# pqh22/ProxyTransformation

Measured on AMD Instinct MI355X. Metric: scenes/sec (100k pts, 256 clusters, 64 proxies), higher is better.
Workload: dtype f32; 1 GPU; cfg2: N=100000 pts, gs=8->M'=256 kept clusters, L=64 text + V=196 image proxies, d=256, eval forward; scenes_per_gpu=4, img_feat_dtype=bf16, input_sets_rotated=3, streams=1, lanes=1 (one forward at a time), setup_forwards=32

## Files before the change

### proxytransformation_amd/csrc/api.hip

```cpp
#include <atomic>
#include <chrono>
#include <cmath>
#include <cstdlib>
#include <cstring>
#include <mutex>
#include <utility>
#include <vector>

#include "common.h"

namespace ptx {

static thread_local char g_err[512] = "";

void set_error(const char *fmt, ...)
{
    va_list ap;
    va_start(ap, fmt);
    vsnprintf(g_err, sizeof(g_err), fmt, ap);
    va_end(ap);
}

static const char *const kKernelNames[] = {
    "k_minmax", "k_cluster", "k_select", "k_tags",
// ... 977 lines not shown
    PTX_REQUIRE(points && tag && kcenter && translate && transform && out && counts, "ptx_affine_compact: null argument");
    PTX_TRY(check_bufs(s, workspace, ws_bytes));
    hipStream_t st = static_cast<hipStream_t>(stream);
    int32_t *tc = at<int32_t>(workspace, ws_layout(*s).tile_counts);
    PTX_TRY(launch_tile_count(tag, s->B, s->N, tc, counts, nullptr, st));
    ScenePts sp;
    PTX_TRY(make_scene_pts(points, nullptr, s->B, s->N, &sp));
    return launch_affine(*s, sp, const_cast<uint32_t *>(tag), kcenter, translate, transform, out, counts, tc, true, false, st);
}

#define PTX_DBG(field, src, bytes)                                                                         do {                                                                                                       if (debug && debug->field)                                                                                 PTX_HIP(hipMemcpyAsync(debug->field, src, bytes, hipMemcpyDeviceToDevice, st));                } while (0)

int ptx_forward(PtxContext *ctx, const PtxShape *s, const PtxWeights *w, const void *prep, const float *lin,
                const float *points, const float *const *points_list, const float *text_feats,
                const uint8_t *text_mask, const void *img_feat, const int32_t *order_override,
                const float *centers_override,
                float *out, int32_t *counts, void *workspace, size_t ws_bytes, const PtxDebug *debug,
                void *stream)
{
    return ptx_forward_ex(ctx, s, w, prep, lin, points, points_list, text_feats, text_mask, img_feat, order_override,
                          centers_override, out, counts, workspace, ws_bytes, debug, nullptr, stream);
}

int ptx_forward_ex(PtxContext *ctx, const PtxShape *s, const PtxWeights *w, const void *prep, const float *lin,
                   const float *points, const float *const *points_list, const float *text_feats,
                   const uint8_t *text_mask, const void *img_feat, const int32_t *order_override,
                   const float *centers_override,
                   float *out, int32_t *counts, void *workspace, size_t ws_bytes, const PtxDebug *debug,
                   const PtxForwardOpts *opts, void *stream)
{
    PTX_REQUIRE(w && prep && lin && (points || points_list) && text_feats && img_feat && out && counts,
                "ptx_forward: null argument");
    const uint32_t *bbox_in = opts ? opts->bbox_enc : nullptr;
    const int compute_dtype = opts ? opts->compute_dtype : 0;
    PTX_REQUIRE(compute_dtype == 0 || compute_dtype == 1, "ptx_forward: compute_dtype=%d (0 fp32-equivalent, 1 bf16)", compute_dtype);
    PTX_TRY(check_bufs(s, workspace, ws_bytes));
    ScenePts sp;
    PTX_TRY(make_scene_pts(points, points_list, s->B, s->N, &sp));
    hipStream_t st = static_cast<hipStream_t>(stream);
    const PtxShape &S = *s;
    const PrepLayout P = prep_layout(S);
    const WsLayout L = ws_layout(S);
    const float *pf = static_cast<const float *>(prep);
    void *ws = workspace;
    const int M = S.grid_size * S.grid_size * S.grid_size, B = S.B, K = S.K, Kd = S.Mt - S.Mk;

    PtxContext *side = ctx;
    if (side == nullptr) PTX_TRY(default_context(&side));
    {
        int dev = 0;
        PTX_HIP(hipGetDevice(&dev));
        PTX_REQUIRE(dev == side->dev, "ptx_forward: context belongs to device %d, current device is %d", side->dev, dev);
    }
    std::lock_guard<std::mutex> enqueue_lock(side->mu);
    hipStreamCaptureStatus cap_status = hipStreamCaptureStatusNone;
    PTX_HIP(hipStreamIsCapturing(st, &cap_status));
    const bool capturing = cap_status != hipStreamCaptureStatusNone;
    if (!capturing) {
        PTX_TRY(gate_check(side));
        side->last_st = st; side->have_last = true;
        if (side->gates_on && (!side->probed || side->probed_st != st)) PTX_TRY(gate_probe(side, st));
    }
    const LayoutChoice lc = choose_layout(S);
    const double est_cluster = lc.est_cluster, est_image = lc.est_image;
    const LayoutForce &lf = lc.lf;
    const bool cluster_on_caller = lc.cluster_on_caller;
    hipStream_t cs = cluster_on_caller ? st : side->st, is = cluster_on_caller ? side->st : st;
    const bool gated = side->gates_on && !cluster_on_caller && !capturing;
    const bool img_late = lc.img_late;
    if (!gated && !img_late) {
        PTX_HIP(hipEventRecord(side->fork, st));
        PTX_HIP(hipStreamWaitEvent(side->st, side->fork, 0));
    }
    float *img_proxy = at<float>(ws, L.img_proxy);
#ifdef PTX_TEST_HOOKS
    static const char *const fault = getenv("PTX_GATE_FAULT");
#else
    constexpr const char *fault = nullptr;
#endif
    const bool fault_fork = gated && fault && fault[0] == 'f', fault_join = gated && fault && fault[0] == 'j';
    auto launch_gate = [&](int kid, hipStream_t s_, const GateRef &g) -> int {
        hipLaunchKernelGGL(k_gate, dim3(1), dim3(64), 0, s_, g);
        PTX_LAUNCHED("k_gate");
        (void)kid;
        return PTX_OK;
    };
    if (gated) {
        const uint32_t seq = ++side->gate_seq;
        PTX_TRY(run_img_proxy(S, *w, pf, img_feat, img_proxy, ws, is, 1, true, 0, -1, fault_fork ? nullptr : side->gate, seq));
        PTX_TIMED(KID_GATE_FORK, cs, launch_gate(KID_GATE_FORK, cs, gate_ref(side, 0, seq, 1)));
    } else
    if (!img_late) PTX_TRY(run_img_proxy(S, *w, pf, img_feat, img_proxy, ws, is, 1));

    uint32_t *mm_ws = at<uint32_t>(ws, L.mm_enc), *tag = at<uint32_t>(ws, L.tag);
    const uint32_t *mm_enc = bbox_in ? bbox_in : mm_ws;
    const bool dbg = debug != nullptr;
    float *centers0 = dbg && debug->centers0 ? at<float>(ws, L.centers0) : nullptr;
    float *cluster1 = dbg && debug->cluster1 ? at<float>(ws, L.cluster1) : nullptr;
    float *offsets = dbg && debug->offsets ? at<float>(ws, L.offsets) : nullptr;
    float *centers = at<float>(ws, L.centers), *cluster2 = at<float>(ws, L.cluster2);
    int32_t *idx2 = at<int32_t>(ws, L.idx2), *pad_count = at<int32_t>(ws, L.pad_count);
    if (!bbox_in) PTX_TIMED(KID_MINMAX, cs, launch_minmax(sp, B, S.N, mm_ws, cs));
    const bool early = lc.early;
    const bool fork_ext = !capturing && (img_late || early);
    const bool cgate = cluster_on_caller && side->gates_on && side->lo_ok && !capturing;
    if (cgate) ++side->gate_seq;
    const bool fault_cjoin = cgate && fault && fault[0] == 'j', fault_ctags = cgate && fault && fault[0] == 't';
    const bool cg_join_select = cgate && early;
    const bool cg_join_qkv = cgate && !early;
    GateRef cjoin = (cg_join_select || cg_join_qkv) ? gate_ref(side, 52, side->gate_seq, 2) : GateRef{};
    PTX_TIMED(KID_CLUSTER, cs, launch_cluster(S, mm_enc, lin, sp, pf + P.off_ab, w->offset, w->offset_map_w,
                                              centers_override, nullptr, centers0, cluster1, offsets, centers, idx2,
                                              cluster2, pad_count, cs, fork_ext ? side->early_a : nullptr));

    if (img_late) {
        if (!fork_ext) PTX_HIP(hipEventRecord(side->fork, st));
        PTX_HIP(hipStreamWaitEvent(side->st, fork_ext ? side->early_a : side->fork, 0));
        PTX_TRY(run_img_proxy(S, *w, pf, img_feat, img_proxy, ws, is, 1));
    }
    float *point_proxy = at<float>(ws, L.point_proxy);
    float *xin_t = at<float>(ws, L.x_in[0]), *xin_i = at<float>(ws, L.x_in[1]);
    float *translate = at<float>(ws, L.head[0]), *transform = at<float>(ws, L.head[1]);
    float *guide_t = (debug && debug->text_guide) ? at<float>(ws, L.guide[0]) : nullptr;
    float *guide_i = (debug && debug->img_guide) ? at<float>(ws, L.guide[1]) : nullptr;
    Branch br[2] = {make_branch(S, *w, pf, 0, xin_t, text_feats, S.L, text_mask, translate, guide_t),
                    make_branch(S, *w, pf, 1, xin_i, at<float>(ws, L.cbuf), S.V, nullptr, transform, guide_i)};
    br[1].proxy_lnp = at<float>(ws, L.lnp_img);
    if (early) {
        if (!fork_ext) PTX_HIP(hipEventRecord(side->early_a, cs));
        PTX_HIP(hipStreamWaitEvent(side->lo, side->early_a, 0));
        float *pp_all = at<float>(ws, L.pp_all), *xa_t = at<float>(ws, L.xln_all[0]), *xa_i = at<float>(ws, L.xln_all[1]);
        int32_t *order_e = at<int32_t>(ws, L.order_e);
        PTX_TRY(launch_order(S, pad_count, order_override, order_e, side->lo));
        PTX_TRY(launch_pointnet(pf + P.enc_ab, w->encoder, centers, cluster2, B * S.Mt, S.Mt, K, S.C, pp_all, &w->text, &w->img, nullptr,
                                nullptr, xa_t, xa_i, S.ln_eps, order_e, M, side->lo, nullptr, 0, true));
        GemmBatch g{}; g.n = 2;
        g.p[0] = GemmProb{xa_t, w->text.qkv_w, at<float>(ws, L.g_all[0]), nullptr, nullptr, nullptr, nullptr, B * S.Mt, 3 * S.C, S.C, S.C, S.C,
                          3 * S.C, 0, 0, 0, EPI_NONE};
        g.p[1] = GemmProb{xa_i, w->img.qkv_w, at<float>(ws, L.g_all[1]), nullptr, nullptr, nullptr, nullptr, B * S.Mt, 3 * S.C, S.C, S.C, S.C,
                          3 * S.C, 0, 0, 0, EPI_NONE};
        PTX_TRY(launch_gemm(g, side->lo, compute_dtype));
        PTX_TRY(run_blocks(S, br, 2, point_proxy, ws, side->lo, 1, compute_dtype, nullptr, nullptr, true));
    }

    int32_t *order = at<int32_t>(ws, L.order), *picks = at<int32_t>(ws, L.picks), *keep = at<int32_t>(ws, L.keep);
    float *kcenter = at<float>(ws, L.kcenter);
    float *kcluster = dbg && debug->kcluster ? at<float>(ws, L.kcluster) : nullptr;
    int32_t *kidx = dbg && debug->kidx ? at<int32_t>(ws, L.kidx) : nullptr;
    int32_t *drop_idx = dbg && debug->drop_idx ? at<int32_t>(ws, L.drop_idx) : nullptr;
    int32_t *ksrc = at<int32_t>(ws, L.ksrc);
    const bool ext_event = !capturing;
    const bool tags_gated = gated && side->lo_ok && (lf.v[3] >= 0 ? lf.v[3] != 0 : est_image < 1.6 * est_cluster);
    const bool tags_tail = !cluster_on_caller && !tags_gated;
    PTX_TIMED(KID_SELECT, cs, launch_select_order(S, centers, pad_count, order_override, order, picks, keep, kcenter,
                                                  ksrc, bbox_in ? nullptr : mm_ws, cs, cluster_on_caller, ext_event && !tags_tail ? side->aux : nullptr,
                                                  cg_join_select ? &cjoin : nullptr));
    int32_t *tile_counts = at<int32_t>(ws, L.tile_counts);
    hipStream_t ts = tags_tail ? cs : side->lo;
    const bool slots_first = !cluster_on_caller && !tags_tail;
    auto enqueue_tags = [&]() -> int {
        if (tags_gated) {
            PTX_TIMED(KID_GATE_TAGS, ts, launch_gate(KID_GATE_TAGS, ts, gate_ref(side, 36, side->gate_seq, 6)));
        } else if (!tags_tail) {
            if (!ext_event) PTX_HIP(hipEventRecord(side->aux, cs));
            PTX_HIP(hipStreamWaitEvent(ts, side->aux, 0));
        }
        if (kcluster || kidx || drop_idx)
            PTX_TRY(launch_select_slots(S, idx2, cluster2, order, picks, keep, kcluster, kidx, drop_idx, nullptr, ts));
        PTX_TIMED(KID_TAGS, ts, launch_tags(S, idx2, order, picks, ksrc, tag, tile_counts, counts, at<int32_t>(ws, L.scene_acc), ts));
        if (tags_gated) {
            auto sig = [&]() -> int {
                hipLaunchKernelGGL(k_signal, dim3(1), dim3(64), 0, ts, side->gate + 38, side->gate_seq);
                PTX_LAUNCHED("k_signal[tags]");
                return PTX_OK;
            };
            PTX_TIMED(KID_SIGNAL_TAGS, ts, sig());
        } else if (cgate) {
            if (!fault_ctags) {
                hipLaunchKernelGGL(k_signal, dim3(1), dim3(64), 0, ts, side->gate + 56, side->gate_seq);
                PTX_LAUNCHED("k_signal[ctags]");
            }
        } else if (!tags_tail) PTX_HIP(hipEventRecord(side->tags, ts));
        return PTX_OK;
    };
    if (slots_first) PTX_TRY(enqueue_tags());

    const bool want_img_proxy = debug != nullptr && debug->img_proxy != nullptr;
    PTX_TRY(run_img_proxy(S, *w, pf, img_feat, img_proxy, ws, is, 2, want_img_proxy));

    bool joined_early = false;
    if (early) {
        const float *const gsrc[2] = {at<float>(ws, L.g_all[0]), at<float>(ws, L.g_all[1])};
        const float *const tb[2] = {pf + P.qkvb[0], pf + P.qkvb[1]};
        float *const qk[2] = {at<float>(ws, L.qkv[0]), at<float>(ws, L.qkv[1])};
        {
            PTX_TRY(run_blocks(S, br, 2, point_proxy, ws, is, 3, compute_dtype));
            PTX_HIP(hipEventRecord(side->join, is));
            PTX_HIP(hipStreamWaitEvent(side->lo, side->join, 0));
            joined_early = true;
        }
        if (cg_join_select) {
            if (!fault_cjoin) {
                hipLaunchKernelGGL(k_signal, dim3(1), dim3(64), 0, side->lo, side->gate + 52, side->gate_seq);
                PTX_LAUNCHED("k_signal[cjoin]");
            }
        } else {
            PTX_HIP(hipEventRecord(side->early_b, side->lo));
            PTX_HIP(hipStreamWaitEvent(cs, side->early_b, 0));
        }
        PTX_TIMED(KID_POINTNET, cs, launch_qkv_gather(at<float>(ws, L.pp_all), gsrc, tb, keep, B, S.Mt, S.Mk, S.C, point_proxy, qk, cs));
    } else
    PTX_TIMED(KID_POINTNET, cs, launch_pointnet(pf + P.enc_ab, w->encoder, kcenter, cluster2, B * S.Mk, S.Mk, K,
                                                S.C, point_proxy, &w->text, &w->img, pf + P.posb_t, pf + P.posb_i, xin_t,
                                                xin_i, S.ln_eps, ksrc, M, cs, tags_gated ? side->gate + 36 : nullptr, side->gate_seq));
    if (!slots_first && !tags_tail) PTX_TRY(enqueue_tags());

    if (!early) PTX_TRY(run_blocks(S, br, 2, point_proxy, ws, cs, 1, compute_dtype, cg_join_qkv ? &cjoin : nullptr));
    if (cg_join_qkv && cjoin.flag != nullptr) {
        set_error("ptx_forward: the join gate was not attached to the qkv launch");
        return PTX_ELAUNCH;
    }
    if (tags_tail) PTX_TRY(enqueue_tags());
    const bool pp_early = cluster_on_caller;
    GateRef join{};
    if (gated) {
        auto launch_signal = [&]() -> int {
            hipLaunchKernelGGL(k_signal, dim3(1), dim3(64), 0, cs, side->gate + 32, side->gate_seq);
            PTX_LAUNCHED("k_signal");
            return PTX_OK;
        };
        if (!fault_join) PTX_TIMED(KID_SIGNAL_JOIN, cs, launch_signal());
        join = gate_ref(side, 32, side->gate_seq, 2);
    } else {
    if (!cluster_on_caller) PTX_HIP(hipEventRecord(side->join, cs));
    if (pp_early && !joined_early) PTX_TRY(run_blocks(S, br, 2, point_proxy, ws, is, 3, compute_dtype));
    if (cg_join_qkv) {
        if (!fault_cjoin) {
            hipLaunchKernelGGL(k_signal, dim3(1), dim3(64), 0, is, side->gate + 52, side->gate_seq);
            PTX_LAUNCHED("k_signal[cjoin]");
        }
    } else {
    if (cluster_on_caller && !joined_early) PTX_HIP(hipEventRecord(side->join, is));
    if (!joined_early) PTX_HIP(hipStreamWaitEvent(st, side->join, 0));
    }
    }
    GateRef tags_join{};
    if (tags_gated) tags_join = gate_ref(side, 38, side->gate_seq, 7);
    if (cgate) tags_join = gate_ref(side, 56, side->gate_seq, 7);
    PTX_TRY(run_blocks(S, br, 2, point_proxy, ws, st, pp_early ? 4 : 2, compute_dtype, &join, &tags_join));
    if (join.flag != nullptr) {
        set_error("ptx_forward: the join gate was not attached to a launch");
        return PTX_ELAUNCH;
    }

    if (cgate && tags_join.flag != nullptr) {
        set_error("ptx_forward: the tags gate was not attached to the proj launch");
        return PTX_ELAUNCH;
    }
    if (!tags_tail && !tags_gated && !cgate) PTX_HIP(hipStreamWaitEvent(st, side->tags, 0));
    PTX_DBG(tag, tag, (size_t)B * S.N * 4);
    PTX_TIMED(KID_AFFINE, st, launch_affine(S, sp, tag, kcenter, translate, transform, out, counts, tile_counts,
                                            true, true, st, (gated || cgate) ? side->gate + 48 : nullptr));

    PTX_DBG(centers0, centers0, (size_t)B * M * 3 * 4);
    PTX_DBG(cluster1, cluster1, (size_t)B * M * K * 3 * 4);
    PTX_DBG(offsets, offsets, (size_t)B * M * 3 * 4);
    PTX_DBG(centers, centers, (size_t)B * M * 3 * 4);
    PTX_DBG(cluster2, cluster2, (size_t)B * M * K * 3 * 4);
    PTX_DBG(idx2, idx2, (size_t)B * M * K * 4);
    PTX_DBG(pad_count, pad_count, (size_t)B * M * 4);
    PTX_DBG(order, order, (size_t)B * S.Mt * 4);
    PTX_DBG(picks, picks, (size_t)B * Kd * 4);
    PTX_DBG(keep, keep, (size_t)B * S.Mk * 4);
    PTX_DBG(kidx, kidx, (size_t)B * S.Mk * K * 4);
    PTX_DBG(drop_idx, drop_idx, (size_t)B * Kd * K * 4);
    PTX_DBG(kcenter, kcenter, (size_t)B * S.Mk * 3 * 4);
    PTX_DBG(kcluster, kcluster, (size_t)B * S.Mk * K * 3 * 4);
    PTX_DBG(point_proxy, point_proxy, (size_t)B * S.Mk * S.C * 4);
    PTX_DBG(img_proxy, img_proxy, (size_t)B * S.V * S.C * 4);
    PTX_DBG(text_guide, guide_t, (size_t)B * S.Mk * S.C * 4);
    PTX_DBG(img_guide, guide_i, (size_t)B * S.Mk * S.C * 4);
    PTX_DBG(translate, translate, (size_t)B * S.Mk * 3 * 4);
    PTX_DBG(transform, transform, (size_t)B * S.Mk * 9 * 4);
    return PTX_OK;
}

}
```

### proxytransformation_amd/csrc/cluster.hip

```cpp
#include <cstdlib>
#include <hip/hip_ext.h>

#include "common.h"

namespace ptx {

__global__ __launch_bounds__(256) void k_minmax(ScenePts points, int N,
                                                uint32_t *__restrict__ mm_enc)
{
    __shared__ float red[4][6];
    minmax_block<false>(points.p[blockIdx.y], N, mm_enc, blockIdx.y, blockIdx.x, gridDim.x, red);
}

int launch_minmax(const ScenePts &points, int B, int N, uint32_t *mm_enc, hipStream_t st)
{
    hipLaunchKernelGGL(k_minmax, dim3(minmax_chunks(N), B), dim3(256), 0, st, points, N, mm_enc);
    PTX_LAUNCHED("k_minmax");
    return PTX_OK;
}

constexpr int kBqUnroll = 4;

__device__ __forceinline__ void grid_centre(const uint32_t *__restrict__ mm_enc, const float *__restrict__ lin, int gs,
                                            float margin, int b, int m, float (&mn)[3], float (&mx)[3], float (&c)[3])
// ... 586 lines not shown
                    const f32x2 d2 = (dx * dx + dy * dy) + dz * dz;
#pragma unroll
                    for (int e = 0; e < 2; ++e) {
                        const int i = 2 * j + e;
                        const uint32_t u = min(mind[i], __float_as_uint(d2[e]));
                        mind[i] = u;
                        if (u > bv) { bv = u; bi = i; }
                    }
                }
            } else {
#pragma unroll
                for (int i = 0; i < P; ++i) {
                    const float d2 = dist2_nofma(lx, ly, lz, px[i][0], py[i][0], pz[i][0]);
                    const uint32_t u = min(mind[i], __float_as_uint(d2));
                    mind[i] = u;
                    if (u > bv) { bv = u; bi = i; }
                }
            }
            uint32_t g = bv;
            g = max(g, (uint32_t)__builtin_amdgcn_update_dpp(0, (int)g, 0x128, 0xf, 0xf, false));
            g = max(g, (uint32_t)__builtin_amdgcn_update_dpp(0, (int)g, 0x124, 0xf, 0xf, false));
            g = max(g, (uint32_t)__builtin_amdgcn_update_dpp(0, (int)g, 0x122, 0xf, 0xf, false));
            g = max(g, (uint32_t)__builtin_amdgcn_update_dpp(0, (int)g, 0x121, 0xf, 0xf, false));
            const uint32_t gmax = max(max((uint32_t)__builtin_amdgcn_readlane((int)g, 0), (uint32_t)__builtin_amdgcn_readlane((int)g, 16)),
                                      max((uint32_t)__builtin_amdgcn_readlane((int)g, 32), (uint32_t)__builtin_amdgcn_readlane((int)g, 48)));
            const unsigned long long who = __ballot(bv == gmax);
            const int leader = __ffsll((long long)who) - 1;
            const int cand = ((ONE ? 0 : wid * 64) + leader) * P + __builtin_amdgcn_readlane(bi, leader);
            if (ONE) {
                last = cand;
                if (lane == 0) s_picks[k] = last;
                continue;
            }
            const int par = (k & 1) * 4;
            if (lane == 0) s_cand[par + wid] = make_uint2(~(uint32_t)cand, gmax);
            __syncthreads();
            const unsigned long long *cw = reinterpret_cast<const unsigned long long *>(s_cand + par);
            const unsigned long long bw = max(max(cw[0], cw[1]), max(cw[2], cw[3]));
            last = (int)~(uint32_t)bw;
            if (tid == 0) s_picks[k] = last;
        }
        __builtin_amdgcn_s_setprio(0);
    }
    __syncthreads();
    for (int k = tid; k < Kd; k += T) {
        const int pk = k < kn ? s_picks[k] : -1;
        a.picks[(size_t)b * Kd + k] = pk;
        if (pk >= 0) s_flag[pk] = 1;
    }
    __syncthreads();

    if (wid == 0) {
        const unsigned long long lt = (1ull << lane) - 1ull;
        int n = 0;
        for (int t0 = 0; t0 < Mt && n < Mk; t0 += 64) {
            const int t = t0 + lane;
            const bool kp = t < Mt && s_flag[t] == 0;
            const unsigned long long mask = __ballot(kp);
            const int pos = n + __popcll(mask & lt);
            if (kp && pos < Mk) s_keep[pos] = t;
            n += __popcll(mask);
        }
    }
    __syncthreads();

    if (a.mm_clear != nullptr && tid < 6) a.mm_clear[b * 6 + tid] = 0u;
    for (int j = tid; j < Mk; j += T) {
        const int t = s_keep[j];
        a.keep[(size_t)b * Mk + j] = t;
        if (a.ksrc != nullptr) a.ksrc[(size_t)b * Mk + j] = s_order[t];
        a.kcenter[((size_t)b * Mk + j) * 3] = sx[t];
        a.kcenter[((size_t)b * Mk + j) * 3 + 1] = sy[t];
        a.kcenter[((size_t)b * Mk + j) * 3 + 2] = sz[t];
    }
    if (a.tail.flag != nullptr && b == 0 && tid == 0) gate_wait(a.tail);
}

__global__ __launch_bounds__(256) void k_select_slots(SelectArgs a)
{
    const int b = blockIdx.y;
    const int M = a.M, K = a.K, Mt = a.Mt, Mk = a.Mk, Kd = a.Kd;
    const int e = blockIdx.x * 256 + threadIdx.x;
    const int kn = Kd < Mt ? Kd : Mt;
    uint32_t *tag = a.tag ? a.tag + (size_t)b * a.N : nullptr;
    const int32_t *order = a.order + (size_t)b * Mt;
    if (e < Mk * K) {
        const int j = e / K, k = e - j * K;
        const int src = order[a.keep[(size_t)b * Mk + j]];
        const int id = a.idx[((size_t)b * M + src) * K + k];
        if (a.kidx) a.kidx[(size_t)b * Mk * K + e] = id;
        if (a.kcluster) {
            const float *cp = a.cluster + (((size_t)b * M + src) * K + k) * 3;
            float *op = a.kcluster + ((size_t)b * Mk * K + e) * 3;
            op[0] = cp[0]; op[1] = cp[1]; op[2] = cp[2];
        }
        if (tag && id >= 0) {
            const uint32_t v = (uint32_t)(e + 1);
            const uint32_t old = atomicMax(&tag[id], v);
            if (old & 0x80000000u) atomicMax(&tag[id], 0x80000000u | v);
        }
    } else if (e < (Mk + Kd) * K) {
        const int ed = e - Mk * K;
        const int kk = ed / K, k = ed - kk * K;
        const int pk = kk < kn ? a.picks[(size_t)b * Kd + kk] : -1;
        int id = -1;
        if (pk >= 0) id = a.idx[((size_t)b * M + order[pk]) * K + k];
        if (a.drop_idx) a.drop_idx[(size_t)b * Kd * K + ed] = id;
        if (tag && id >= 0) atomicOr(&tag[id], 0x80000000u);
    }
}

static size_t select_lds_bytes(const PtxShape &s)
{
    const int Kd = s.Mt - s.Mk;
    return sizeof(int) * ((size_t)s.Mt * 5 + s.Mk + (Kd > 0 ? Kd : 1) + 64 + 16 + 16);
}

static SelectArgs select_args(const PtxShape &s, const int32_t *idx, const float *centers, const float *cluster,
                              const int32_t *pad_count, const int32_t *order_override, int32_t *order,
                              int32_t *picks, int32_t *keep, float *kcenter, float *kcluster, int32_t *kidx,
                              int32_t *drop_idx, uint32_t *tag, uint32_t *mm_clear)
{
    return SelectArgs{idx, centers, cluster, pad_count, order_override, order, picks, keep, kcenter,
                      kcluster, kidx, drop_idx, tag, s.grid_size * s.grid_size * s.grid_size, s.K, s.Mt,
                      s.Mk, s.Mt - s.Mk, s.N, nullptr, mm_clear, GateRef{}};
}

int launch_select_order(const PtxShape &s, const float *centers, const int32_t *pad_count,
                        const int32_t *order_override, int32_t *order, int32_t *picks, int32_t *keep,
                        float *kcenter, int32_t *ksrc, uint32_t *mm_clear, hipStream_t st, bool critical,
                        hipEvent_t done, const GateRef *tail)
{
    SelectArgs a = select_args(s, nullptr, centers, nullptr, pad_count, order_override, order, picks, keep, kcenter,
                               nullptr, nullptr, nullptr, nullptr, mm_clear);
    a.ksrc = ksrc;
    if (tail != nullptr) a.tail = *tail;
    size_t lds = select_lds_bytes(s);
    PTX_REQUIRE(lds <= 160 * 1024, "select: Mt=%d needs %zu B of LDS (> 160 KiB)", s.Mt, lds);
    const bool alone = critical;
    if (alone && s.B <= 32 && lds < 150 * 1024) lds = 150 * 1024;
    const bool one = critical && s.Mt <= 384;
    const int per = cdiv(s.Mt, one ? 64 : 256);
    const dim3 grid(s.B), block(256);
#define PTX_SEL(P_)                                                                          \
    do {                                                                                     \
        if (lds > 64 * 1024) {                                                               \
            PTX_HIP(hipFuncSetAttribute(reinterpret_cast<const void *>(&k_select<P_, false>), \
                                        hipFuncAttributeMaxDynamicSharedMemorySize, (int)lds)); \
            if (one && P_ <= 6)                                                              \
                PTX_HIP(hipFuncSetAttribute(reinterpret_cast<const void *>(&k_select<(P_ <= 6 ? P_ : 1), true>), \
                                            hipFuncAttributeMaxDynamicSharedMemorySize, (int)lds)); \
        }                                                                                    \
         \
        if (one && P_ <= 6) hipExtLaunchKernelGGL((k_select<(P_ <= 6 ? P_ : 1), true>), grid, block, lds, st, nullptr, done, 0, a); \
        else hipExtLaunchKernelGGL((k_select<P_, false>), grid, block, lds, st, nullptr, done, 0, a); \
    } while (0)
    if (per <= 1) PTX_SEL(1);
    else if (per <= 2) PTX_SEL(2);
    else if (per <= 3) PTX_SEL(3);
    else if (per <= 4) PTX_SEL(4);
    else if (per <= 5) PTX_SEL(5);
    else if (per <= 6) PTX_SEL(6);
    else if (per <= 8) PTX_SEL(8);
    else if (per <= 12) PTX_SEL(12);
    else if (per <= 16) PTX_SEL(16);
    else { set_error("select: Mt=%d too large (max %d)", s.Mt, 256 * 16); return PTX_EINVAL; }
#undef PTX_SEL
    PTX_LAUNCHED("k_select");
    return PTX_OK;
}

int launch_select_slots(const PtxShape &s, const int32_t *idx, const float *cluster, const int32_t *order,
                        const int32_t *picks, const int32_t *keep, float *kcluster, int32_t *kidx,
                        int32_t *drop_idx, uint32_t *tag, hipStream_t st)
{
    SelectArgs a = select_args(s, idx, nullptr, cluster, nullptr, nullptr, const_cast<int32_t *>(order),
                               const_cast<int32_t *>(picks), const_cast<int32_t *>(keep), nullptr, kcluster, kidx,
                               drop_idx, tag, nullptr);
    hipLaunchKernelGGL(k_select_slots, dim3(cdiv(s.Mt * s.K, 256), s.B), dim3(256), 0, st, a);
    PTX_LAUNCHED("k_select_slots");
    return PTX_OK;
}

int launch_select(const PtxShape &s, const int32_t *idx, const float *centers, const float *cluster,
                  const int32_t *pad_count, const int32_t *order_override, int32_t *order,
                  int32_t *picks, int32_t *keep, float *kcenter, float *kcluster, int32_t *kidx,
                  int32_t *drop_idx, uint32_t *tag, hipStream_t st)
{
    PTX_TRY(launch_select_order(s, centers, pad_count, order_override, order, picks, keep, kcenter, nullptr, nullptr, st, true, nullptr));
    PTX_TRY(launch_select_slots(s, idx, cluster, order, picks, keep, kcluster, kidx, drop_idx, nullptr, st));
    if (tag == nullptr) return PTX_OK;
    return launch_tags(s, idx, order, picks, nullptr, tag, nullptr, nullptr, nullptr, st, keep);
}

__global__ __launch_bounds__(256) void k_tile_count(const uint32_t *__restrict__ tag, int N,
                                                    int32_t *__restrict__ tile_counts, int32_t *scene_acc,
                                                    int32_t *counts)
{
    const int b = blockIdx.y, tile = blockIdx.x;
    const uint32_t *tg = tag + (size_t)b * N;
    int c = 0;
#pragma unroll
    for (int r = 0; r < kTilePts / 256; ++r) {
        const int n = tile * kTilePts + r * 256 + threadIdx.x;
        if (n < N) c += (tg[n] >> 31) == 0;
    }
    c = wave_sum(c);
    __shared__ int red[4];
    if (lane_id() == 0) red[threadIdx.x >> 6] = c;
    __syncthreads();
    if (threadIdx.x == 0) {
        const int total = red[0] + red[1] + red[2] + red[3];
        tile_counts[b * gridDim.x + tile] = total;
        if (scene_acc != nullptr) {
            __hip_atomic_fetch_add(scene_acc + 2 * b, total, __ATOMIC_RELAXED, __HIP_MEMORY_SCOPE_AGENT);
            const int ticket = __hip_atomic_fetch_add(scene_acc + 2 * b + 1, 1, __ATOMIC_ACQ_REL, __HIP_MEMORY_SCOPE_AGENT);
            if (ticket == (int)gridDim.x - 1) {
                const int sum = __hip_atomic_exchange(scene_acc + 2 * b, 0, __ATOMIC_ACQUIRE, __HIP_MEMORY_SCOPE_AGENT);
                __hip_atomic_store(scene_acc + 2 * b + 1, 0, __ATOMIC_RELAXED, __HIP_MEMORY_SCOPE_AGENT);
                __hip_atomic_store(counts + b, sum, __ATOMIC_RELEASE, __HIP_MEMORY_SCOPE_SYSTEM);
            }
        }
    }
}

struct TagArgs {
    const int32_t *idx, *order, *picks, *ksrc;
    const int32_t *keep;
    uint32_t *tag; int32_t *tile_counts, *scene_acc, *counts;
    int M, K, Mt, Mk, Kd, N, ntiles;
};

template <int TILES>
__global__ __launch_bounds__(1024) void k_tags(TagArgs a)
{
    constexpr int kTagRange = TILES * kTilePts;
    extern __shared__ __attribute__((aligned(16))) uint32_t s_tag[];
    int *s_cnt = reinterpret_cast<int *>(s_tag + kTagRange);
    const int b = blockIdx.y, base = blockIdx.x * kTagRange, tid = threadIdx.x;
    const int M = a.M, K = a.K, Mt = a.Mt, Mk = a.Mk, Kd = a.Kd;
    const int kn = Kd < Mt ? Kd : Mt;
    for (int i = tid * 4; i < kTagRange; i += 1024 * 4) *reinterpret_cast<uint4 *>(s_tag + i) = make_uint4(0u, 0u, 0u, 0u);
    if (tid < TILES) s_cnt[tid] = 0;
    __syncthreads();
    const int32_t *idx = a.idx + (size_t)b * M * K;
    const int32_t *order = a.order + (size_t)b * Mt;
    for (int e0 = tid; e0 < Mk * K; e0 += 4 * 1024) {
        int id[4];
#pragma unroll
        for (int u = 0; u < 4; ++u) {
            const int e = e0 + u * 1024;
            const int ec = min(e, Mk * K - 1), j = ec / K, k = ec - j * K;
            const int src = a.ksrc != nullptr ? a.ksrc[(size_t)b * Mk + j] : order[a.keep[(size_t)b * Mk + j]];
            id[u] = e < Mk * K ? idx[(size_t)src * K + k] : -1;
        }
#pragma unroll
        for (int u = 0; u < 4; ++u) {
            const unsigned r = (unsigned)(id[u] - base);
            if (r < (unsigned)kTagRange) atomicMax(&s_tag[r], (uint32_t)(e0 + u * 1024 + 1));
        }
    }
    __syncthreads();
    for (int e0 = tid; e0 < Kd * K; e0 += 4 * 1024) {
        int id[4];
#pragma unroll
        for (int u = 0; u < 4; ++u) {
            const int ed = e0 + u * 1024;
            const int ec = min(ed, Kd * K - 1), kk = ec / K, k = ec - kk * K;
            const int pk = (ed < Kd * K && kk < kn) ? a.picks[(size_t)b * Kd + kk] : -1;
            id[u] = pk >= 0 ? idx[(size_t)order[pk] * K + k] : -1;
        }
#pragma unroll
        for (int u = 0; u < 4; ++u) {
            const unsigned r = (unsigned)(id[u] - base);
            if (r < (unsigned)kTagRange) atomicOr(&s_tag[r], 0x80000000u);
        }
    }
    __syncthreads();
    uint32_t *tg = a.tag + (size_t)b * a.N;
    const int lim = min(kTagRange, a.N - base);
    const bool vec = ((a.N & 3) == 0);
    for (int i0 = 0; i0 < lim; i0 += 1024 * 4) {
        const int i = i0 + tid * 4;
        int c = 0;
        if (i < lim) {
            const uint4 v = *reinterpret_cast<const uint4 *>(s_tag + i);
            if (vec) {
                *reinterpret_cast<uint4 *>(tg + base + i) = v;
                c = (int)((v.x >> 31) == 0) + (int)((v.y >> 31) == 0) + (int)((v.z >> 31) == 0) + (int)((v.w >> 31) == 0);
            } else {
                const uint32_t w[4] = {v.x, v.y, v.z, v.w};
#pragma unroll
                for (int q = 0; q < 4; ++q)
                    if (i + q < lim) { tg[base + i + q] = w[q]; c += (int)((w[q] >> 31) == 0); }
            }
        }
        c = wave_sum(c);
        if (lane_id() == 0 && i < kTagRange) atomicAdd(&s_cnt[i / kTilePts], c);
    }
    __syncthreads();
    const int t0 = blockIdx.x * TILES;
    if (a.tile_counts != nullptr && tid < TILES && t0 + tid < a.ntiles) a.tile_counts[b * a.ntiles + t0 + tid] = s_cnt[tid];
    if (tid == 0 && a.scene_acc != nullptr) {
        int total = 0;
        for (int t = 0; t < TILES; ++t) total += s_cnt[t];
        __hip_atomic_fetch_add(a.scene_acc + 2 * b, total, __ATOMIC_RELAXED, __HIP_MEMORY_SCOPE_AGENT);
        const int ticket = __hip_atomic_fetch_add(a.scene_acc + 2 * b + 1, 1, __ATOMIC_ACQ_REL, __HIP_MEMORY_SCOPE_AGENT);
        if (ticket == (int)gridDim.x - 1) {
            const int sum = __hip_atomic_exchange(a.scene_acc + 2 * b, 0, __ATOMIC_ACQUIRE, __HIP_MEMORY_SCOPE_AGENT);
            __hip_atomic_store(a.scene_acc + 2 * b + 1, 0, __ATOMIC_RELAXED, __HIP_MEMORY_SCOPE_AGENT);
            __hip_atomic_store(a.counts + b, sum, __ATOMIC_RELEASE, __HIP_MEMORY_SCOPE_SYSTEM);
        }
    }
}

int launch_tags(const PtxShape &s, const int32_t *idx, const int32_t *order, const int32_t *picks, const int32_t *ksrc,
                uint32_t *tag, int32_t *tile_counts, int32_t *counts, int32_t *scene_acc, hipStream_t st, const int32_t *keep)
{
    const int M = s.grid_size * s.grid_size * s.grid_size;
    TagArgs a{idx, order, picks, ksrc, keep, tag, tile_counts, scene_acc, counts, M, s.K, s.Mt, s.Mk, s.Mt - s.Mk, s.N,
              cdiv(s.N, kTilePts)};
    const bool small = (long)s.B * cdiv(s.N, 16 * kTilePts) < 16;
    if (small) {
        const size_t lds = sizeof(uint32_t) * 4 * kTilePts + 16 * sizeof(int);
        hipLaunchKernelGGL(k_tags<4>, dim3(cdiv(s.N, 4 * kTilePts), s.B), dim3(1024), lds, st, a);
    } else {
        const size_t lds = sizeof(uint32_t) * 16 * kTilePts + 16 * sizeof(int);
        PTX_HIP(hipFuncSetAttribute(reinterpret_cast<const void *>(&k_tags<16>), hipFuncAttributeMaxDynamicSharedMemorySize, (int)lds));
        hipLaunchKernelGGL(k_tags<16>, dim3(cdiv(s.N, 16 * kTilePts), s.B), dim3(1024), lds, st, a);
    }
    PTX_LAUNCHED("k_tags");
    return PTX_OK;
}

__global__ __launch_bounds__(64) void k_scene_counts(const int32_t *tile_counts, int ntiles, int32_t *counts)
{
    const int b = blockIdx.x;
    int c = 0;
    for (int t = threadIdx.x; t < ntiles; t += 64) c += tile_counts[b * ntiles + t];
    c = wave_sum(c);
    if (threadIdx.x == 0) {
        __hip_atomic_store(counts + b, c, __ATOMIC_RELEASE, __HIP_MEMORY_SCOPE_SYSTEM);
    }
}

int launch_tile_count(const uint32_t *tag, int B, int N, int32_t *tile_counts, int32_t *counts, int32_t *scene_acc,
                      hipStream_t st)
{
    const int ntiles = cdiv(N, kTilePts);
    hipLaunchKernelGGL(k_tile_count, dim3(ntiles, B), dim3(256), 0, st, tag, N, tile_counts,
                       counts ? scene_acc : nullptr, counts);
    PTX_LAUNCHED("k_tile_count");
    if (counts && scene_acc == nullptr) {
        hipLaunchKernelGGL(k_scene_counts, dim3(B), dim3(64), 0, st, tile_counts, ntiles, counts);
        PTX_LAUNCHED("k_scene_counts");
    }
    return PTX_OK;
}

struct AffineArgs {
    ScenePts points; uint32_t *tag; const float *kcenter, *translate, *transform;
    float *out; int32_t *counts; const int32_t *tile_counts; int N, Mk, K;
    int clear_tag;
    const uint32_t *poison;
};

template <bool COMPACT, bool TABLE>
__global__ __launch_bounds__(256) void k_affine(AffineArgs a)
{
    extern __shared__ float s_tab[];
    const int b = blockIdx.y, tile = blockIdx.x, ntiles = gridDim.x;
    const int tid = threadIdx.x, lane = lane_id(), wid = tid >> 6;
    uint32_t *tg = a.tag + (size_t)b * a.N;
    const float *__restrict__ pts = a.points.p[b];
    float *out = a.out + (size_t)b * a.N * 3;
    constexpr int R = kTilePts / 256;
    __shared__ int s_cnt[R][4];
    __shared__ int s_base;
    __shared__ uint32_t s_poison;
    const float *kc = a.kcenter + (size_t)b * a.Mk * 3, *kT = a.transform + (size_t)b * a.Mk * 9, *kt = a.translate + (size_t)b * a.Mk * 3;
    int acc = 0;
    if (COMPACT) acc = a.tile_counts[b * ntiles + min(tid, ntiles - 1)];
    if (tid == 0) s_poison = a.poison != nullptr ? __hip_atomic_load(a.poison, __ATOMIC_RELAXED, __HIP_MEMORY_SCOPE_AGENT) : 0u;
    constexpr int kBatch = 8;
    const int c3 = 3 * a.Mk, c12 = 12 * a.Mk, c15 = 15 * a.Mk;
    auto tab_src = [&](int i) {
        const float *p = i < c3 ? kc + i : i < c12 ? kT + (i - c3) : kt + (i - c12);
        return *p;
    };
    constexpr int kAhead = 4;
    float tb[kAhead][kBatch];
    if (TABLE) {
#pragma unroll
        for (int h = 0; h < kAhead; ++h)
            if (h * kBatch * 256 < c15) {
#pragma unroll
                for (int u = 0; u < kBatch; ++u) tb[h][u] = tab_src(min((h * kBatch + u) * 256 + tid, c15 - 1));
            }
    }
    uint32_t tgv[R]; float v[R][3];
#pragma unroll
    for (int r = 0; r < R; ++r) {
        const int nc = min(tile * kTilePts + r * 256 + tid, a.N - 1);
        tgv[r] = tg[nc];
        v[r][0] = pts[(size_t)nc * 3]; v[r][1] = pts[(size_t)nc * 3 + 1]; v[r][2] = pts[(size_t)nc * 3 + 2];
    }
    if (TABLE) {
#pragma unroll
        for (int h = 0; h < kAhead; ++h)
#pragma unroll
            for (int u = 0; u < kBatch; ++u) {
                const int i = (h * kBatch + u) * 256 + tid;
                if (i < c15) s_tab[i] = tb[h][u];
            }
        for (int i0 = kAhead * kBatch * 256; i0 < c15; i0 += kBatch * 256) {
            float t2[kBatch];
#pragma unroll
            for (int u = 0; u < kBatch; ++u) t2[u] = tab_src(min(i0 + u * 256 + tid, c15 - 1));
#pragma unroll
            for (int u = 0; u < kBatch; ++u) {
                const int i = i0 + u * 256 + tid;
                if (i < c15) s_tab[i] = t2[u];
            }
        }
    }
    int base = 0;
    if (COMPACT) {
        acc = tid < tile ? acc : 0;
        for (int t = tid + 256; t < tile; t += 256) acc += a.tile_counts[b * ntiles + t];
        acc = wave_sum(acc);
        if (lane == 0) s_cnt[0][wid] = acc;
    }
    __syncthreads();
    if (s_poison != 0u) {
#pragma unroll
        for (int r = 0; r < R; ++r) {
            const int n = tile * kTilePts + r * 256 + tid;
            if (n < a.N) { out[(size_t)n * 3] = out[(size_t)n * 3 + 1] = out[(size_t)n * 3 + 2] = __uint_as_float(0x7fc00000u); }
        }
        return;
    }
    if (COMPACT) {
        base = s_cnt[0][0] + s_cnt[0][1] + s_cnt[0][2] + s_cnt[0][3];
        __syncthreads();
    }
    (void)s_base;
    bool keep[R]; unsigned long long bal[R];
#pragma unroll
    for (int r = 0; r < R; ++r) {
        const int n = tile * kTilePts + r * 256 + tid;
        keep[r] = false;
        if (n < a.N) {
            const uint32_t t = tgv[r];
            if (a.clear_tag && t != 0u) tg[n] = 0u;
            float x = v[r][0], y = v[r][1], z = v[r][2];
            keep[r] = !COMPACT || (t >> 31) == 0;
            const uint32_t own = t & 0x7fffffffu;
            if (own != 0 && keep[r]) {
                const int j = (int)(own - 1) / a.K;
                float c[3], T[9], tr[3];
                if (TABLE) {
#pragma unroll
                    for (int d = 0; d < 3; ++d) { c[d] = s_tab[3 * j + d]; tr[d] = s_tab[c12 + 3 * j + d]; }
#pragma unroll
                    for (int d = 0; d < 9; ++d) T[d] = s_tab[c3 + 9 * j + d];
                } else {
#pragma unroll
                    for (int d = 0; d < 3; ++d) { c[d] = kc[3 * j + d]; tr[d] = kt[3 * j + d]; }
#pragma unroll
                    for (int d = 0; d < 9; ++d) T[d] = kT[9 * j + d];
                }
                const float dx = x - c[0], dy = y - c[1], dz = z - c[2];
                const float rx = fmaf(T[2], dz, fmaf(T[1], dy, T[0] * dx));
                const float ry = fmaf(T[5], dz, fmaf(T[4], dy, T[3] * dx));
                const float rz = fmaf(T[8], dz, fmaf(T[7], dy, T[6] * dx));
                x = (rx + c[0]) + tr[0]; y = (ry + c[1]) + tr[1]; z = (rz + c[2]) + tr[2];
            }
            v[r][0] = x; v[r][1] = y; v[r][2] = z;
        }
        bal[r] = __ballot(keep[r]);
        if (COMPACT && lane == 0) s_cnt[r][wid] = __popcll(bal[r]);
    }
    if (!COMPACT) {
// ... 43 lines not shown
```

Baseline: 18540 scenes/s.

## Prefetch tag indices before LDS clear and adapt tag tile count to grid size

The k_tags kernel now issues its first rounds of dependent index loads (own/keep and drop picks through order into idx) into registers before clearing shared memory, so global load latency overlaps the LDS clear and barrier. The ksrc/keep choice becomes a template parameter. Tiles per block are chosen adaptively among 4, 8 and 16 to cap the grid near a target group count. Select skips the hipExtLaunch completion event when no consumer needs it. This adds register pressure and a more complex launch dispatch.

```diff
diff --git a/proxytransformation_amd/csrc/api.hip b/proxytransformation_amd/csrc/api.hip
--- a/proxytransformation_amd/csrc/api.hip
+++ b/proxytransformation_amd/csrc/api.hip
@@ -1153,8 +1153,9 @@
     const bool ext_event = !capturing;
     const bool tags_gated = gated && side->lo_ok && (lf.v[3] >= 0 ? lf.v[3] != 0 : est_image < 1.6 * est_cluster);
     const bool tags_tail = !cluster_on_caller && !tags_gated;
+    hipEvent_t select_done = ext_event && !tags_tail && !tags_gated ? side->aux : nullptr;
     PTX_TIMED(KID_SELECT, cs, launch_select_order(S, centers, pad_count, order_override, order, picks, keep, kcenter,
-                                                  ksrc, bbox_in ? nullptr : mm_ws, cs, cluster_on_caller, ext_event && !tags_tail ? side->aux : nullptr,
+                                                  ksrc, bbox_in ? nullptr : mm_ws, cs, cluster_on_caller, select_done,
                                                   cg_join_select ? &cjoin : nullptr));
     int32_t *tile_counts = at<int32_t>(ws, L.tile_counts);
     hipStream_t ts = tags_tail ? cs : side->lo;
diff --git a/proxytransformation_amd/csrc/cluster.hip b/proxytransformation_amd/csrc/cluster.hip
--- a/proxytransformation_amd/csrc/cluster.hip
+++ b/proxytransformation_amd/csrc/cluster.hip
@@ -762,7 +762,11 @@
                                             hipFuncAttributeMaxDynamicSharedMemorySize, (int)lds)); \
         }                                                                                    \
          \
-        if (one && P_ <= 6) hipExtLaunchKernelGGL((k_select<(P_ <= 6 ? P_ : 1), true>), grid, block, lds, st, nullptr, done, 0, a); \
+         \
+        if (done == nullptr) {                                                               \
+            if (one && P_ <= 6) hipLaunchKernelGGL((k_select<(P_ <= 6 ? P_ : 1), true>), grid, block, lds, st, a); \
+            else hipLaunchKernelGGL((k_select<P_, false>), grid, block, lds, st, a);         \
+        } else if (one && P_ <= 6) hipExtLaunchKernelGGL((k_select<(P_ <= 6 ? P_ : 1), true>), grid, block, lds, st, nullptr, done, 0, a); \
         else hipExtLaunchKernelGGL((k_select<P_, false>), grid, block, lds, st, nullptr, done, 0, a); \
     } while (0)
     if (per <= 1) PTX_SEL(1);
@@ -841,7 +845,9 @@
     int M, K, Mt, Mk, Kd, N, ntiles;
 };
 
-template <int TILES>
+constexpr int kTagOwn = 8, kTagDrop = 4;
+
+template <int TILES, bool THRU>
 __global__ __launch_bounds__(1024) void k_tags(TagArgs a)
 {
     constexpr int kTagRange = TILES * kTilePts;
@@ -850,19 +856,67 @@
     const int b = blockIdx.y, base = blockIdx.x * kTagRange, tid = threadIdx.x;
     const int M = a.M, K = a.K, Mt = a.Mt, Mk = a.Mk, Kd = a.Kd;
     const int kn = Kd < Mt ? Kd : Mt;
-    for (int i = tid * 4; i < kTagRange; i += 1024 * 4) *reinterpret_cast<uint4 *>(s_tag + i) = make_uint4(0u, 0u, 0u, 0u);
-    if (tid < TILES) s_cnt[tid] = 0;
-    __syncthreads();
+    const int nown = Mk * K, ndrop = Kd * K;
     const int32_t *idx = a.idx + (size_t)b * M * K;
     const int32_t *order = a.order + (size_t)b * Mt;
-    for (int e0 = tid; e0 < Mk * K; e0 += 4 * 1024) {
+    const int32_t *own = (THRU ? a.keep : a.ksrc) + (size_t)b * Mk;
+    const int32_t *picks = kn > 0 ? a.picks + (size_t)b * Kd : order;
+
+    int oid[kTagOwn], did[kTagDrop];
+    {
+        int o1[kTagOwn], ok[kTagOwn], d1[kTagDrop], dk[kTagDrop];
+        bool dreal[kTagDrop];
+#pragma unroll
+        for (int u = 0; u < kTagOwn; ++u) {
+            const int ec = min(tid + u * 1024, nown - 1), j = ec / K;
+            ok[u] = ec - j * K;
+            o1[u] = own[j];
+        }
+#pragma unroll
+        for (int u = 0; u < kTagDrop; ++u) {
+            const int ec = max(min(tid + u * 1024, ndrop - 1), 0), kk = ec / K;
+            dk[u] = ec - kk * K;
+            dreal[u] = tid + u * 1024 < ndrop && kk < kn;
+            d1[u] = picks[min(kk, max(kn - 1, 0))];
+        }
+        for (int i = tid * 4; i < kTagRange; i += 1024 * 4) *reinterpret_cast<uint4 *>(s_tag + i) = make_uint4(0u, 0u, 0u, 0u);
+        if (tid < TILES) s_cnt[tid] = 0;
+        if (THRU) {
+#pragma unroll
+            for (int u = 0; u < kTagOwn; ++u) o1[u] = order[o1[u]];
+        }
+#pragma unroll
+        for (int u = 0; u < kTagDrop; ++u) {
+            const bool real = dreal[u] && d1[u] >= 0;
+            const int src = order[min(max(d1[u], 0), Mt - 1)];
+            d1[u] = real ? src : -1;
+        }
+#pragma unroll
+        for (int u = 0; u < kTagOwn; ++u) {
+            const int id = idx[(size_t)o1[u] * K + ok[u]];
+            oid[u] = tid + u * 1024 < nown ? id : -1;
+        }
+#pragma unroll
+        for (int u = 0; u < kTagDrop; ++u) {
+            const int id = idx[(size_t)max(d1[u], 0) * K + dk[u]];
+            did[u] = d1[u] >= 0 ? id : -1;
+        }
+    }
+    __syncthreads();
+#pragma unroll
+    for (int u = 0; u < kTagOwn; ++u) {
+        const unsigned r = (unsigned)(oid[u] - base);
+        if (r < (unsigned)kTagRange) atomicMax(&s_tag[r], (uint32_t)(tid + u * 1024 + 1));
+    }
+    for (int e0 = tid + kTagOwn * 1024; e0 < nown; e0 += 4 * 1024) {
         int id[4];
 #pragma unroll
         for (int u = 0; u < 4; ++u) {
             const int e = e0 + u * 1024;
-            const int ec = min(e, Mk * K - 1), j = ec / K, k = ec - j * K;
-            const int src = a.ksrc != nullptr ? a.ksrc[(size_t)b * Mk + j] : order[a.keep[(size_t)b * Mk + j]];
-            id[u] = e < Mk * K ? idx[(size_t)src * K + k] : -1;
+            const int ec = min(e, nown - 1), j = ec / K, k = ec - j * K;
+            const int src = THRU ? order[own[j]] : own[j];
+            const int v = idx[(size_t)src * K + k];
+            id[u] = e < nown ? v : -1;
         }
 #pragma unroll
         for (int u = 0; u < 4; ++u) {
@@ -871,14 +925,20 @@
         }
     }
     __syncthreads();
-    for (int e0 = tid; e0 < Kd * K; e0 += 4 * 1024) {
+#pragma unroll
+    for (int u = 0; u < kTagDrop; ++u) {
+        const unsigned r = (unsigned)(did[u] - base);
+        if (r < (unsigned)kTagRange) atomicOr(&s_tag[r], 0x80000000u);
+    }
+    for (int e0 = tid + kTagDrop * 1024; e0 < ndrop; e0 += 4 * 1024) {
         int id[4];
 #pragma unroll
         for (int u = 0; u < 4; ++u) {
             const int ed = e0 + u * 1024;
-            const int ec = min(ed, Kd * K - 1), kk = ec / K, k = ec - kk * K;
-            const int pk = (ed < Kd * K && kk < kn) ? a.picks[(size_t)b * Kd + kk] : -1;
-            id[u] = pk >= 0 ? idx[(size_t)order[pk] * K + k] : -1;
+            const int ec = min(ed, ndrop - 1), kk = ec / K, k = ec - kk * K;
+            const int pk = picks[min(kk, kn - 1)];
+            const int v = idx[(size_t)order[min(max(pk, 0), Mt - 1)] * K + k];
+            id[u] = ((ed < ndrop) & (kk < kn) & (pk >= 0)) ? v : -1;
         }
 #pragma unroll
         for (int u = 0; u < 4; ++u) {
@@ -924,21 +984,34 @@
     }
 }
 
+constexpr long kTagGroupsMax = 64;
+
 int launch_tags(const PtxShape &s, const int32_t *idx, const int32_t *order, const int32_t *picks, const int32_t *ksrc,
                 uint32_t *tag, int32_t *tile_counts, int32_t *counts, int32_t *scene_acc, hipStream_t st, const int32_t *keep)
 {
     const int M = s.grid_size * s.grid_size * s.grid_size;
     TagArgs a{idx, order, picks, ksrc, keep, tag, tile_counts, scene_acc, counts, M, s.K, s.Mt, s.Mk, s.Mt - s.Mk, s.N,
               cdiv(s.N, kTilePts)};
-    const bool small = (long)s.B * cdiv(s.N, 16 * kTilePts) < 16;
-    if (small) {
-        const size_t lds = sizeof(uint32_t) * 4 * kTilePts + 16 * sizeof(int);
-        hipLaunchKernelGGL(k_tags<4>, dim3(cdiv(s.N, 4 * kTilePts), s.B), dim3(1024), lds, st, a);
-    } else {
-        const size_t lds = sizeof(uint32_t) * 16 * kTilePts + 16 * sizeof(int);
-        PTX_HIP(hipFuncSetAttribute(reinterpret_cast<const void *>(&k_tags<16>), hipFuncAttributeMaxDynamicSharedMemorySize, (int)lds));
-        hipLaunchKernelGGL(k_tags<16>, dim3(cdiv(s.N, 16 * kTilePts), s.B), dim3(1024), lds, st, a);
-    }
+    PTX_REQUIRE(ksrc != nullptr || keep != nullptr, "tags: neither ksrc nor keep");
+    int tiles = 4;
+    while (tiles < 16 && (long)s.B * cdiv(s.N, tiles * kTilePts) > kTagGroupsMax) tiles *= 2;
+    const size_t lds = sizeof(uint32_t) * tiles * kTilePts + 16 * sizeof(int);
+    const dim3 grid(cdiv(s.N, tiles * kTilePts), s.B), block(1024);
+    const bool thru = ksrc == nullptr;
+#define PTX_TAGS(T_)                                                                          \
+    do {                                                                                      \
+         \
+        if (lds > 64 * 1024) {                                                                \
+            PTX_HIP(hipFuncSetAttribute(reinterpret_cast<const void *>(&k_tags<T_, false>), hipFuncAttributeMaxDynamicSharedMemorySize, (int)lds)); \
+            PTX_HIP(hipFuncSetAttribute(reinterpret_cast<const void *>(&k_tags<T_, true>), hipFuncAttributeMaxDynamicSharedMemorySize, (int)lds)); \
+        }                                                                                     \
+        if (thru) hipLaunchKernelGGL((k_tags<T_, true>), grid, block, lds, st, a);            \
+        else hipLaunchKernelGGL((k_tags<T_, false>), grid, block, lds, st, a);                \
+    } while (0)
+    if (tiles == 4) PTX_TAGS(4);
+    else if (tiles == 8) PTX_TAGS(8);
+    else PTX_TAGS(16);
+#undef PTX_TAGS
     PTX_LAUNCHED("k_tags");
     return PTX_OK;
 }
```

Result: no change. 18510 scenes/s, median of 3 (-0.1%).
